# iris-ua/iris_lama

Hardware: AMD Instinct MI355X
Metric: particle-scans/sec (higher is better)
Workload: dtype f64; 1 GPU; PFSlam2D 30 particles, 1080-beam synthetic corridor log (SURVEY.md 8(d)), res 0.05 m, patch 32, l2_max 0.5, GN+Cauchy(0.15), seed 42; particles=30, beams=1080, parallelism=particle-shard x1

## Files before the change

### iris_lama_amd/csrc/lama_dev.h

```cpp
#pragma once
#include <hip/hip_runtime.h>
#include <stdint.h>
#include <cstddef>

#ifdef LAMA_WIDE_DM
#define lama_dev lama_dev_wide
#endif

#include "lama_heap.h"

#ifdef LAMA_WAVE_SIM
#define LAMA_LOCKSTEP() ((void)__ballot(true))
#else
#define LAMA_LOCKSTEP() ((void)0)
#endif

namespace lama_dev {

#ifdef LAMA_WIDE_DM
typedef uint32_t sv_t;
constexpr uint32_t SV_VALID = 0x80000000u;
constexpr uint32_t SV_QUEUED = 0x40000000u;
constexpr uint32_t SV_SQMASK = 0x3FFFFFFFu;
constexpr int SV_VALID_BIT = 31;
constexpr uint32_t MAX_OFFSET_CELLS = 255;
#else
typedef uint16_t sv_t;
constexpr uint16_t SV_VALID = 0x8000;
constexpr uint16_t SV_QUEUED = 0x4000;
constexpr uint16_t SV_SQMASK = 0x3FFF;
constexpr int SV_VALID_BIT = 15;
constexpr uint32_t MAX_OFFSET_CELLS = 127;
#endif
constexpr uint32_t SV_BYTES = (uint32_t)sizeof(sv_t);
constexpr uint32_t SV_PATCH_BYTES = 1024u * SV_BYTES;

// ... 25 lines not shown
    uint32_t qcap;
    const PartRec* part;
    uint32_t max_sqdist;
    uint32_t max_iter;
    double scale, off, resolution, maxdist, meas_sigma;
    double trunc_ray, trunc_range;
    int16_t* dm_dir;
    int16_t* occ_dir;
    int32_t* counts;
    double* poses;
    uint64_t* q_lower;
    uint64_t* q_raise;
    uint32_t* qsizes;
    uint32_t* slow;
    uint32_t* slow_list;
    uint32_t* slow_n;
    uint8_t* heavy;
    const uint32_t* elist;
    const uint32_t* elist_n;
    const uint8_t* early;
    uint32_t lane;
    uint64_t* act;
    uint32_t* act_count;
    uint32_t act_cap;
    uint64_t* stats;
    int32_t* err;
    uint64_t* dbg;
    uint32_t* guard;
    uint32_t guard_r;
    uint32_t occ_policy, ray_rule;
    uint32_t strategy;
    double lo_miss, lo_hit, lo_min, lo_max;
};

struct PV {
    int16_t* dm_dir; int16_t* occ_dir;
    sv_t* dm_sv; uint32_t* dm_obs; uint64_t* dm_mask;
    uint32_t* occ; uint64_t* occ_mask; uint64_t* occ_hit;
    int32_t* counts; int32_t* rev;
    uint32_t dm_cap, occ_cap;
};
#ifdef LAMA_WAVE_SIM
__device__ inline uint32_t part_u32(const uint32_t* q) { return *q; }
__device__ inline uint64_t part_u64(const uint64_t* q) { return *q; }
#else
__device__ inline uint32_t part_u32(const uint32_t* q)
{
    return (uint32_t)__builtin_amdgcn_readfirstlane((int)__hip_atomic_load(q, __ATOMIC_RELAXED, __HIP_MEMORY_SCOPE_AGENT));
}
__device__ inline uint64_t part_u64(const uint64_t* q)
{
    const uint64_t v = __hip_atomic_load(q, __ATOMIC_RELAXED, __HIP_MEMORY_SCOPE_AGENT);
    const uint32_t lo = (uint32_t)__builtin_amdgcn_readfirstlane((int)(uint32_t)v), hi = (uint32_t)__builtin_amdgcn_readfirstlane((int)(uint32_t)(v >> 32));
    return ((uint64_t)hi << 32) | lo;
}
#endif
#if defined(LAMA_KC_PROBE) && !defined(LAMA_WAVE_SIM)
__device__ uint32_t g_kc_n;
__device__ uint64_t g_kc_ev[64][8];
__device__ __noinline__ void kc_probe(const DevParams& prm, int p)
{
    const uint64_t* q = reinterpret_cast<const uint64_t*>(prm.part + p);
#if LAMA_KC_PROBE == 2
    __builtin_amdgcn_s_dcache_inv();
#endif
    const unsigned long long act = __ballot(1);
// ... 423 lines not shown
```

### iris_lama_amd/csrc/lama_hip.hip

```cpp
#include "../../include/lama_hip.h"

#include <hip/hip_runtime.h>

#include <algorithm>
#include <cmath>
#include <cstdio>
#include <cstdlib>
#include <cstring>
#include <map>
#include <memory>
#include <mutex>
#include <string>
#include <vector>

#include "lama_kernels.h"
#include "lama_pgo.h"
#include "lama_pgo_pcg.h"
#include "lama_map_build.h"
#include "lama_match_batch.h"
#include "lama_correlative.h"
#include "../host/pgo_pattern.hpp"

using namespace lama_dev;

// ... 841 lines not shown
    return regrid_window(c, (uint32_t)newW, nox, noy);
}

int32_t start_without_first_scan(lama_hip_ctx* c)
{
    if (c->initialised) return LAMA_HIP_OK;
    for (uint32_t p = 0; p < c->P; ++p) { c->h_poses[4 * p] = 1.0; c->h_poses[4 * p + 1] = 0.0; c->h_poses[4 * p + 2] = 0.0; c->h_poses[4 * p + 3] = 0.0; }
    HIPCHK(c, hipMemcpyAsync(c->d_poses, c->h_poses.data(), sizeof(double) * 4 * c->P, hipMemcpyHostToDevice, c->stream));
    c->initialised = true;
    return LAMA_HIP_OK;
}

int32_t fit_window(lama_hip_ctx* c, const Affine& mtf, uint32_t first, uint32_t count)
{
    double far = c->scan_reach;
    if (c->cfg.ray_rule == 0 && c->cfg.truncated_range > 0.0) far = std::min(far, c->cfg.truncated_range);
    const uint32_t guard_r = ((uint32_t)std::ceil(std::sqrt((double)c->max_sqdist)) + 1u + 31u) / 32u;
    const double reach = far + std::sqrt(mtf.t[0] * mtf.t[0] + mtf.t[1] * mtf.t[1]) + (double)(guard_r + 1u) * 32.0 * c->cfg.resolution;
    double xlo = 1e300, xhi = -1e300, ylo = 1e300, yhi = -1e300;
    for (uint32_t p = first; p < first + count; ++p) {
        const double x = c->h_poses[4 * p + 2], y = c->h_poses[4 * p + 3];
        xlo = std::min(xlo, x - reach); xhi = std::max(xhi, x + reach);
        ylo = std::min(ylo, y - reach); yhi = std::max(yhi, y + reach);
    }
    auto patch = [&](double w) { return (int64_t)std::floor((c->scale * w + c->off) / 32.0); };
    return ensure_window(c, patch(xlo), patch(xhi), patch(ylo), patch(yhi));
}

static unsigned xcd_grid(const lama_hip_ctx* c, uint32_t first, uint32_t count)
{
    return first + count == c->P ? (count + 7u) / 8u * 8u : count;
}

int32_t launch_allocation_phase(lama_hip_ctx* c, const DevParams& prm, uint32_t n, uint32_t first, uint32_t count, int alloc_only, hipStream_t s, const double* d_pts)
{
    const size_t need = (size_t)c->P * n;
    if (need > c->d_rrec.n) {
        c->d_rrec.reset(); c->d_rbbox.reset(); c->d_rchunk.reset();
        hipError_t e = c->d_rrec.alloc(need);
        if (e == hipSuccess) e = c->d_rbbox.alloc(need);
        if (e == hipSuccess) e = c->d_rchunk.alloc((size_t)c->P * ((n + 63) / 64));
        if (e != hipSuccess) { c->d_rrec.reset(); return hip_fail(c, e, "ray buffers"); }
    }
    hipLaunchKernelGGL(k_ray_hits, dim3(xcd_grid(c, first, count), (n + 255) / 256), dim3(256), 0, s, prm, d_pts, (int)n, c->d_tfs, (int)first,
                       c->d_rrec, c->d_rbbox, alloc_only, c->d_rchunk);
    const int rw_seg = count <= 64 ? 4 : 1;
    hipLaunchKernelGGL(k_ray_alloc_walk, dim3(xcd_grid(c, first, count), (n * rw_seg + 255) / 256), dim3(256), 0, s, prm, (const lama_dev::RayRec*)c->d_rrec, (int)n, (int)first, rw_seg);
    double far = c->scan_reach;
    if (c->cfg.truncated_range > 0.0) far = std::min(far, c->cfg.truncated_range);
    const int reach_cells = (int)std::ceil(far * c->scale) + 2;
    hipLaunchKernelGGL(k_occ_reverse_dir, dim3(count), dim3(256), 0, s, prm, (int)first, (const double*)c->d_tfs, reach_cells,
                       c->unguarded_retry ? 1 : 0);
    return LAMA_HIP_OK;
}

static uint32_t route_places(const lama_hip_ctx* c, uint32_t count)
{
    const uint32_t slots = c->num_cus * 12u;
    if (c->route_forced || count >= slots) return c->route_cap;
    return std::min<uint32_t>(c->route_cap, std::max<uint32_t>(8u, (slots - count) / 7u));
}

int32_t run_update_maps(lama_hip_ctx* c, uint32_t n, const Affine& mtf, uint32_t first, uint32_t count, StepGroup* g)
{
    hipStream_t s = g ? g->s : (hipStream_t)c->stream;
    const double* d_pts = g ? (const double*)g->d_pts : (const double*)c->d_pts;
    if (!g) {
        const int32_t rcw = fit_window(c, mtf, first, count);
        if (rcw) return rcw;
        c->last_mtf = mtf; c->last_first = first; c->last_count = count;
        if (c->recover_depth == 0) { c->saved_visit_bound = c->visit_bound; c->saved_ctr = c->ctr; }
    }
    PinVec<double>& tfs = c->h_tfs;
    tfs.resize((size_t)c->P * 12);
    for (uint32_t p = first; p < first + count; ++p) host_scan_tf(&c->h_poses[4 * p], mtf, &tfs[12 * (size_t)p]);
    HIPCHK(c, hipMemcpyAsync(c->d_tfs + 12 * (size_t)first, &tfs[12 * (size_t)first], sizeof(double) * 12 * count, hipMemcpyHostToDevice, s));
    DevParams prm = g ? group_params(c, *g) : make_params(c);
    bool early_lane = false;
    {
        Timer t = g ? Timer(c, g, 1) : Timer(c, &c->ctr.ms_raycast, &c->ctr.launches_raycast);
        if (first == 0 && count == c->P && !g) {
            (void)hipMemsetAsync(c->d_slow_n, 0, 32 + sizeof(uint64_t) * 4 * c->P, c->stream);
        } else {
            (void)hipMemsetAsync(prm.slow_n, 0, 32, s);
            (void)hipMemsetAsync(c->d_stats + 4 * (size_t)first, 0, sizeof(uint64_t) * 4 * count, s);
        }
        bool sequential = c->cfg.sequential_raycast == 1 || c->cfg.occupancy_policy == 1 ||
                          c->cfg.ray_rule == 1;
        if (!sequential && (n > 4096u || (uint64_t)n + 4096u > c->cfg.active_capacity)) sequential = true;
        if (!g && !sequential && (uint64_t)c->visit_bound + n >= 65536u) {
            uint32_t m = 0;
            if (c->initialised) {
                (void)hipMemsetAsync(c->d_scalar, 0, sizeof(uint32_t), c->stream);
                hipLaunchKernelGGL(k_occ_max_visited, dim3(c->P), dim3(256), 0, c->stream, prm, c->d_scalar);
                HIPCHK(c, hipMemcpyAsync(&m, c->d_scalar, sizeof(uint32_t), hipMemcpyDeviceToHost, c->stream));
                HIPCHK(c, hipStreamSynchronize(c->stream));
            }
            c->visit_bound = m;
            if ((uint64_t)m + n >= 65536u) { sequential = true; c->ctr.wrap_guard_scans += 1; }
        }
        if (!g) {
            c->visit_bound = (uint32_t)std::min<uint64_t>((uint64_t)c->visit_bound + n, 65535u);
            if (sequential) c->ctr.sequential_raycast_scans += 1; else c->ctr.parallel_raycast_scans += 1;
        }
        if (!g) c->last_guarded = c->cfg.ray_rule == 0;
        if (!g && !c->last_guarded) {
            const double side = 32.0 * c->cfg.resolution;
            const double rp = c->scan_reach / side + 2.5;
            const uint32_t bound = (uint32_t)std::min(32767.0, std::ceil(3.1416 * rp * rp));
            std::vector<CapRequest> reqs;
            for (uint32_t p = first; p < first + count; ++p) {
                const HostPart& pr = c->h_part[p];
                const uint32_t nd = std::min<uint32_t>(MAX_PATCHES, round_up32((uint32_t)c->h_counts[2 * p] + bound)), no = std::min<uint32_t>(MAX_PATCHES, round_up32((uint32_t)c->h_counts[2 * p + 1] + bound));
                if (nd > pr.dm_cap || no > pr.occ_cap) reqs.push_back(CapRequest{p, std::max(nd, pr.dm_cap), std::max(no, pr.occ_cap)});
            }
            if (!reqs.empty()) {
                const int32_t rg = set_capacities(c, reqs);
                if (rg) return rg;
                prm = make_params(c);
            }
        }
        if (sequential) {
            if (c->last_guarded) { const int32_t ra = launch_allocation_phase(c, prm, n, first, count, 1, c->stream, c->d_pts); if (ra) return ra; }
            hipLaunchKernelGGL(k_raycast, dim3(count), dim3(UM_BLOCK), 0, c->stream, prm, c->d_pts, (int)n, c->d_tfs, (int)first);
        } else {
            const bool two_waves_e = c->cfg.brushfire_waves == 2 || (c->cfg.brushfire_waves == 0 && count <= BF_TW_MAX_PARTICLES);
            early_lane = c->early_on && two_waves_e && c->cfg.brushfire_mode == 0 && first == 0 && count == c->P &&
                         count >= std::max<uint32_t>(c->route_min_count, c->early_min_count) && c->route_cap > 0;
            uint32_t host_n = 0;
            if (early_lane && c->ll_valid) {
                const uint32_t places = route_places(c, count);
                double mean = 0; for (uint32_t p = 0; p < c->P; ++p) mean += c->h_ll[p]; mean /= c->P;
                const double lim = 2.5 * std::min(mean, 0.0) - 5.0;
                std::vector<std::pair<double, uint32_t>> cand;
                for (uint32_t p = 0; p < c->P; ++p) if (c->h_ll[p] < lim) cand.emplace_back(c->h_ll[p], p);
                if (cand.size() > places) { std::partial_sort(cand.begin(), cand.begin() + places, cand.end()); cand.resize(places); }
                c->h_hlist.resize(256);
                for (auto& e : cand) c->h_hlist[host_n++] = e.second;
                if (host_n) HIPCHK(c, hipMemcpyAsync(c->d_hlist, c->h_hlist.data(), sizeof(uint32_t) * host_n, hipMemcpyHostToDevice, c->stream));
            }
            const bool prev_ok = c->early_ok && c->early_candidates > 0;
            early_lane = early_lane && (host_n > 0 || prev_ok);
            if (early_lane)
                hipLaunchKernelGGL(k_early_list, dim3(1), dim3(256), 0, c->stream, prev_ok ? (const uint8_t*)c->d_heavy : (const uint8_t*)nullptr,
                                   (const uint32_t*)c->d_hlist, host_n, c->d_early, c->d_elist, c->d_slow_n + 4, (int)c->P, route_places(c, count));
            { const int32_t ra = launch_allocation_phase(c, prm, n, first, count, 0, s, d_pts); if (ra) return ra; }
#ifdef LAMA_WAVE_SIM
            const unsigned gy = 4u;
#else
            const unsigned gy = count <= 64 ? 128u : (count >= 1024 ? 8u : 32u);
#endif
            if (early_lane) {
                DevParams pe = prm;
                pe.elist = c->d_elist; pe.elist_n = c->d_slow_n + 4; pe.lane = 1;
                const unsigned eg = route_places(c, count);
                hipLaunchKernelGGL(k_ray_patches, dim3(eg, 128u), dim3(256), 0, c->stream, pe, (const lama_dev::RayRec*)c->d_rrec,
                                   (const uint64_t*)c->d_rbbox, (const lama_dev::RayChunk*)c->d_rchunk, (int)n, 0);
                hipLaunchKernelGGL((k_ray_replay<RP_SORT_SMALL, RP_SORT_SMALL, false, RP_BLOCK_LARGE>), dim3(eg), dim3(RP_BLOCK_LARGE), 0, c->stream, pe, 0);
                hipLaunchKernelGGL((k_ray_replay<8192, 8192, true, RP_BLOCK_LARGE>), dim3(eg), dim3(RP_BLOCK_LARGE), 0, c->stream, pe, 0);
                HIPCHK(c, hipEventRecord(c->ev_alloc, c->stream));
                HIPCHK(c, hipStreamWaitEvent(c->stream3, c->ev_alloc, 0));
                hipLaunchKernelGGL(k_mark_early, dim3(1), dim3(64), 0, c->stream3, pe);
                HIPCHK(c, hipEventRecord(c->ev_go, c->stream3));
                hipLaunchKernelGGL((k_brushfire<LQ_BIG, RQ_BIG, true, true>), dim3(eg), dim3(2 * UM_BLOCK), c->big_stage_pad, c->stream3, pe, 0, 2);
                HIPCHK(c, hipEventRecord(c->ev_early, c->stream3));
                HIPCHK(c, hipStreamWaitEvent(c->stream, c->ev_go, 0));
                prm.early = c->d_early;
            }
            hipLaunchKernelGGL(k_ray_patches, dim3(xcd_grid(c, first, count), gy), dim3(256), 0, s, prm, (const lama_dev::RayRec*)c->d_rrec,
                               (const uint64_t*)c->d_rbbox, (const lama_dev::RayChunk*)c->d_rchunk, (int)n, (int)first);
            const unsigned resume_grid = std::min<unsigned>(count, 256u);
            if (count <= 512) {
                hipLaunchKernelGGL((k_ray_replay<RP_SORT_SMALL, RP_SORT_SMALL, false, RP_BLOCK_LARGE>), dim3(count), dim3(RP_BLOCK_LARGE), 0, s, prm, (int)first);
                hipLaunchKernelGGL((k_ray_replay<8192, 8192, true, RP_BLOCK_LARGE>), dim3(resume_grid), dim3(RP_BLOCK_LARGE), 0, s, prm, (int)first);
            } else {
                hipLaunchKernelGGL((k_ray_replay<RP_SORT_SMALL, RP_SORT_SMALL, false, RP_BLOCK_SMALL>), dim3(count), dim3(RP_BLOCK_SMALL), 0, s, prm, (int)first);
                hipLaunchKernelGGL((k_ray_replay<8192, 8192, true, RP_BLOCK_SMALL>), dim3(resume_grid), dim3(RP_BLOCK_SMALL), 0, s, prm, (int)first);
            }
        }
// ... 109 lines not shown
        Timer t(c, &c->ctr.ms_resample, &c->ctr.launches_resample);
        rc = run_jobs(c, true);
        t.stop();
    }
    if (rc) return rc;
    HIPCHK(c, hipMemcpyAsync(c->ms.counts, c->h_counts.data(), sizeof(int32_t) * 2 * P, hipMemcpyHostToDevice, c->stream));
    HIPCHK(c, hipMemcpyAsync(c->d_poses, c->h_poses.data(), sizeof(double) * 4 * P, hipMemcpyHostToDevice, c->stream));
    HIPCHK(c, hipStreamSynchronize(c->stream));
    resolve_timers(c);
    c->ctr.resample_clones += clones.size();
    c->ctr.resample_bytes += c->clone_bytes;
    return LAMA_HIP_OK;
}

int32_t apply_resample(lama_hip_ctx* c, const int32_t* idx)
{
    c->early_ok = false;
    if (c->ll_valid) { std::vector<double> nl(c->P); for (uint32_t i = 0; i < c->P; ++i) nl[i] = c->h_ll[idx[i]]; c->h_ll.swap(nl); }
    return permute_particles(c, idx);
}

bool step_can_group(const lama_hip_ctx* c, uint32_t n)
{
    return c->step_groups > 1 && c->P < c->route_min_count && c->cfg.brushfire_mode == 0 && c->cfg.sequential_raycast != 1 &&
           c->cfg.occupancy_policy != 1 && c->cfg.ray_rule == 0 && n <= 4096u && (uint64_t)n + 4096u <= c->cfg.active_capacity &&
           (uint64_t)c->visit_bound + n < 65536u;
}

int32_t queue_group_match(lama_hip_ctx* c, StepGroup& g, uint32_t n, const Affine& mtf, bool status_only)
{
    const DevParams prm = group_params(c, g);
    hipStream_t s = g.s;
    const double* const d_pts = g.d_pts;
    const uint32_t* const d_words = g.d_words;
    uint8_t* const d_pack = g.d_pack;
    const int first = (int)g.first, count = (int)g.count;
    if (!status_only) {
        HIPCHK(c, hipMemcpyAsync(c->d_poses + 4 * (size_t)g.first, &c->h_poses[4 * (size_t)g.first], sizeof(double) * 4 * g.count, hipMemcpyHostToDevice, s));
        Timer t(c, &g, 0);
        if (c->max_sqdist > (uint32_t)SM_LUT) hipLaunchKernelGGL(k_scan_match<true>, dim3(count), dim3(SM_BLOCK), 0, s, prm, d_pts, (int)n, mtf, c->d_loglik, c->d_iters, first);
        else hipLaunchKernelGGL(k_scan_match<false>, dim3(count), dim3(SM_BLOCK), 0, s, prm, d_pts, (int)n, mtf, c->d_loglik, c->d_iters, first);
        t.stop();
    }
    hipLaunchKernelGGL(k_pack_group, dim3(1), dim3(64), 0, s, prm, (const double*)c->d_loglik, (const int32_t*)c->d_iters, d_words, first, count, d_pack);
    HIPCHK(c, hipGetLastError());
    HIPCHK(c, hipMemcpyAsync(g.h_pack.data(), d_pack, GroupPack(g.count).bytes, hipMemcpyDeviceToHost, g.s));
    HIPCHK(c, hipEventRecord(g.ev_match, g.s));
    return LAMA_HIP_OK;
}

int32_t recover_group(lama_hip_ctx* c, StepGroup& g, int32_t e)
{
    int32_t rc = wait_for_groups(c);
    if (rc) return rc;
    const size_t o = 4 * (size_t)g.first, m = 4 * (size_t)g.count;
    const std::vector<double> now(c->h_poses.data() + o, c->h_poses.data() + o + m);
    std::memcpy(c->h_poses.data() + o, g.upd_poses.data(), sizeof(double) * m);
    const PinVec<double>& scan = g.upd_slot ? c->h_pts2 : c->h_pts;
    HIPCHK(c, c->d_pts.grow((size_t)3 * g.upd_n, (size_t)3 * 2048));
    HIPCHK(c, hipMemcpyAsync(c->d_pts, scan.data(), sizeof(double) * 3 * g.upd_n, hipMemcpyHostToDevice, c->stream));
    const double reach_now = c->scan_reach;
    c->scan_reach = g.upd_reach; c->last_n = g.upd_n;
    c->last_mtf = g.upd_mtf; c->last_first = g.first; c->last_count = g.count; c->last_guarded = true;
    const uint32_t vb = c->visit_bound;
    const lama_hip_counters before = c->ctr;
    c->saved_visit_bound = vb; c->saved_ctr = c->ctr;
    rc = recover_update(c, e);
    c->visit_bound = vb;
    c->ctr.parallel_raycast_scans = before.parallel_raycast_scans; c->ctr.sequential_raycast_scans = before.sequential_raycast_scans;
    c->ctr.ms_raycast = before.ms_raycast; c->ctr.launches_raycast = before.launches_raycast;
    c->ctr.ms_brushfire = before.ms_brushfire; c->ctr.launches_brushfire = before.launches_brushfire;
    c->ctr.bf_longest_chain_sum = before.bf_longest_chain_sum; c->ctr.bf_longest_chain_last = before.bf_longest_chain_last;
    if (rc == LAMA_HIP_OK) { for (uint32_t p = g.first; p < g.first + g.count; ++p) c->h_chain[p] = c->h_stats[4 * (size_t)p + 3]; c->chain_dirty = true; }
    c->scan_reach = reach_now; c->last_n = 0;
    std::memcpy(c->h_poses.data() + o, now.data(), sizeof(double) * m);
    return rc;
}
// ... 301 lines not shown
    c->wx0 = (px - c->W / 2) * 32;
    c->wy0 = (py - c->W / 2) * 32;
    for (uint32_t p = 0; p < c->P; ++p) std::memcpy(&c->h_poses[4 * p], pose0, sizeof(double) * 4);
    HIPCHK(c, hipMemcpyAsync(c->d_poses, c->h_poses.data(), sizeof(double) * 4 * c->P, hipMemcpyHostToDevice, c->stream));
    int32_t rc = upload_scan(c, pts, n);
    if (rc) return rc;
    const Affine mtf = moving_tf(origin3, quat);
    rc = run_update_maps(c, n, mtf, 0, 1);
    if (rc) return rc;
    rc = check_device_errors(c, true, false);
    if (rc) return rc;
    if (c->P > 1) {
        std::vector<int32_t> idx(c->P, 0);
        rc = permute_particles(c, idx.data());
        if (rc) return rc;
    }
    rc = check_device_errors(c, true, false);
    if (rc) return rc;
    c->initialised = true;
    return LAMA_HIP_OK;
}

int32_t lama_hip_pf_scan_match(lama_hip_ctx* c, const double* pts, uint32_t n, const double* origin3, const double* quat,
                               double* poses_out, double* loglik_out, int32_t* iters_out)
{
    if (!c || !pts || n == 0) return LAMA_HIP_E_INVALID;
    ENTER(c);
    if (!c->initialised) return fail(c, LAMA_HIP_E_STATE, "lama_hip_pf_scan_match before lama_hip_pf_init");
    HIPCHK(c, hipSetDevice(c->cfg.device));
    int32_t rc = upload_scan(c, pts, n);
    if (rc) return rc;
    const Affine mtf = moving_tf(origin3, quat);
    DevParams prm = make_params(c);
    {
        Timer t(c, &c->ctr.ms_scan_match, &c->ctr.launches_scan_match);
        if (c->max_sqdist > (uint32_t)SM_LUT) hipLaunchKernelGGL(k_scan_match<true>, dim3(c->P), dim3(SM_BLOCK), 0, c->stream, prm, c->d_pts, (int)n, mtf, c->d_loglik, c->d_iters, 0);
        else hipLaunchKernelGGL(k_scan_match<false>, dim3(c->P), dim3(SM_BLOCK), 0, c->stream, prm, c->d_pts, (int)n, mtf, c->d_loglik, c->d_iters, 0);
        t.stop();
    }
    HIPCHK(c, hipGetLastError());
    c->h_results.resize(c->results_bytes);
    HIPCHK(c, hipMemcpyAsync(c->h_results.data(), c->d_results, c->results_bytes, hipMemcpyDeviceToHost, c->stream));
    rc = check_device_errors(c, false, c->cfg.profile != 0, true);
    if (rc) return rc;
    const uint8_t* r = c->h_results.data();
    std::memcpy(c->h_poses.data(), r, sizeof(double) * 4 * c->P);
    if (poses_out) std::memcpy(poses_out, r, sizeof(double) * 4 * c->P);
    if (loglik_out) std::memcpy(loglik_out, r + sizeof(double) * 4 * c->P, sizeof(double) * c->P);
    if (iters_out) std::memcpy(iters_out, r + sizeof(double) * 5 * c->P, sizeof(int32_t) * c->P);
    c->h_ll.resize(c->P); std::memcpy(c->h_ll.data(), r + sizeof(double) * 4 * c->P, sizeof(double) * c->P); c->ll_valid = true;
    return LAMA_HIP_OK;
}

int32_t lama_hip_pf_resample(lama_hip_ctx* c, const int32_t* sample_idx)
{
    if (!c || !sample_idx) return LAMA_HIP_E_INVALID;
    if (c->poisoned) return fail(c, LAMA_HIP_E_STATE, "the context ran out of device memory in the middle of a resample and cannot continue");
    if (!c->initialised) return fail(c, LAMA_HIP_E_STATE, "lama_hip_pf_resample before lama_hip_pf_init");
    for (uint32_t i = 0; i < c->P; ++i)
        if (sample_idx[i] < 0 || (uint32_t)sample_idx[i] >= c->P) return fail(c, LAMA_HIP_E_INVALID, "sample_idx out of range");
    if (c->groups_busy && !c->resample_deferred) {
        c->deferred_idx.assign(sample_idx, sample_idx + c->P);
        c->resample_deferred = true;
        return LAMA_HIP_OK;
    }
    ENTER(c);
    HIPCHK(c, hipSetDevice(c->cfg.device));
    return apply_resample(c, sample_idx);
}

// ... 1598 lines not shown
```

### iris_lama_amd/csrc/lama_kernels.h

```cpp
#pragma once
#include "lama_dev.h"

namespace lama_dev {

constexpr int SM_BLOCK = 256;
constexpr int UM_BLOCK = 64;
#ifdef LAMA_TEST_SMALL_QUEUES
constexpr int LQ_SMALL = LAMA_TEST_SMALL_QUEUES, RQ_SMALL = LAMA_TEST_SMALL_QUEUES / 4;
#else
constexpr int LQ_SMALL = 1024, RQ_SMALL = 256;
#endif
constexpr int LQ_BIG = 8192, RQ_BIG = 2048;
constexpr uint32_t BF_TW_MAX_PARTICLES = 1u << 30;

template <int CTRL, int ROW_MASK>
__device__ __forceinline__ double dpp_add(double v)
{
    const uint64_t u = (uint64_t)__double_as_longlong(v);
    const uint32_t lo = (uint32_t)__builtin_amdgcn_update_dpp(0, (int)(uint32_t)u, CTRL, ROW_MASK, 0xF, false);
    const uint32_t hi = (uint32_t)__builtin_amdgcn_update_dpp(0, (int)(uint32_t)(u >> 32), CTRL, ROW_MASK, 0xF, false);
    return v + __longlong_as_double((long long)(((uint64_t)hi << 32) | lo));
}

template <int NV>
// ... 279 lines not shown
                } else {
                    sh.mu = sh.mu * sh.v; sh.v = 2 * sh.v;
                    invalid = true;
                }
                sh.reuse = invalid ? 1 : 0;
            }
            if (invalid) {
                stop = lm ? 0 : 1;
                const double mh[3] = {-sh.h[0], -sh.h[1], -sh.h[2]};
                bool ok = true;
                sh.state = se2_exp_mul(mh, sh.state, ok);
                if (!ok) { if (numeric) *numeric = 1; else atomicOr(prm.err, ERR_NUMERIC); }
                sh.tf = scan_tf(sh.state, mtf);
                sh.have_lin = 0;
            } else {
                for (int k = 0; k < NJ; ++k) sh.tot[k] = sh.tot2[k];
                sh.have_lin = 1;
                sh.lin_is_final = 1;
            }
            sh.ctl[1] = stop;
        }
        ++iter;
        __syncthreads();
        SMT(3);
        if (sh.ctl[1]) break;
    }
#ifdef LAMA_PROFILE_SM
    if (threadIdx.x == 0) for (int k = 0; k < 4; ++k) prm.dbg[8 * blockIdx.x + k] = smp[k];
#endif
    return iter;
}
#undef SMT

template <bool BIGSQ>
__global__ __launch_bounds__(SM_BLOCK) __attribute__((amdgpu_num_vgpr(128))) void k_scan_match(DevParams prm, const double* __restrict__ pts, int n, Affine mtf,
                                                          double* __restrict__ loglik_out, int32_t* __restrict__ iters_out, int first_particle)
{
    __shared__ SMShared sh;
    const int p = first_particle + blockIdx.x;
    const PV pv_ = pview_w(prm, p);
    const int16_t* dir = pv_.dm_dir;
    const sv_t* sv = pv_.dm_sv;
    if (threadIdx.x == 0) {
        sh.state = load_pose(prm.poses + 4 * p);
        sh.tf = scan_tf(sh.state, mtf);
        sh.ctl[0] = 0; sh.ctl[1] = 0;
    }
    sm_build_lut(prm, sh.lut);
    __syncthreads();
    uint32_t evals = 0;
    const uint32_t iter = gn_solve<BIGSQ>(prm, dir, sv, pts, n, mtf, sh, evals);
    double loglik;
    if (sh.lin_is_final) {
        loglik = sh.tot[10];
    } else {
        double a2[2];
        {
            const Affine tf = sh.tf;
            eval_beams_res<BIGSQ>(prm, dir, sv, pts, n, tf, a2, sh.lut);
        }
        block_sum<2>(a2, sh.red, sh.tot2);
        loglik = sh.tot2[1];
    }
    ++evals;
    if (threadIdx.x == 0) {
        double* q = prm.poses + 4 * p;
        q[0] = sh.state.c; q[1] = sh.state.s; q[2] = sh.state.tx; q[3] = sh.state.ty;
        loglik_out[p] = loglik;
        iters_out[p] = (int32_t)iter;
        prm.stats[4 * p + 0] = iter;
        prm.stats[4 * p + 1] = evals;
    }
}

__global__ __launch_bounds__(64) void k_pack_group(DevParams prm, const double* __restrict__ loglik, const int32_t* __restrict__ iters,
                                                    const uint32_t* __restrict__ words, int first_particle, int count, uint8_t* __restrict__ out)
{
    double* o_pose = reinterpret_cast<double*>(out);
    double* o_ll = o_pose + 4 * (size_t)count;
    uint64_t* o_st = reinterpret_cast<uint64_t*>(o_ll + count);
    uint32_t* o_guard = reinterpret_cast<uint32_t*>(o_st + 4 * (size_t)count);
    int32_t* o_cnt = reinterpret_cast<int32_t*>(o_guard + count);
    int32_t* o_it = o_cnt + 2 * (size_t)count;
    uint32_t* o_w = reinterpret_cast<uint32_t*>(o_it + count);
    for (int i = threadIdx.x; i < count; i += 64) {
        const int p = first_particle + i;
        for (int k = 0; k < 4; ++k) { o_pose[4 * i + k] = prm.poses[4 * p + k]; o_st[4 * i + k] = prm.stats[4 * p + k]; }
        o_ll[i] = loglik[p];
        o_guard[i] = prm.guard[p];
        o_cnt[2 * i] = prm.counts[2 * p]; o_cnt[2 * i + 1] = prm.counts[2 * p + 1];
        o_it[i] = iters[p];
    }
    if (threadIdx.x < 16) o_w[threadIdx.x] = words[threadIdx.x];
}

__global__ __launch_bounds__(256) void k_match_eval(DevParams prm, int particle, const double* __restrict__ pts, int n, Affine mtf,
                                                     const double* __restrict__ pose, double* __restrict__ r_out, double* __restrict__ j_out,
                                                     int cell_mode )
{
    __shared__ Affine tfs;
    const PV pv_ = pview_w(prm, particle);
    const int16_t* dir = pv_.dm_dir;
    const sv_t* sv = pv_.dm_sv;
    if (threadIdx.x == 0) tfs = load_scan_tf(pose, mtf);
    __syncthreads();
    const Affine tf = tfs;
    const int i = blockIdx.x * 256 + threadIdx.x;
    if (i >= n) return;
    const double px = pts[3 * i], py = pts[3 * i + 1], pz = pts[3 * i + 2];
    double hx, hy;
    hit_xy(tf, px, py, pz, hx, hy);
    if (cell_mode) { r_out[i] = dm_distance_cell(prm, dir, sv, w2m(prm, hx), w2m(prm, hy)); return; }
    double gx, gy;
    r_out[i] = dm_distance(prm, dir, sv, hx, hy, &gx, &gy);
    if (j_out) { j_out[i] = gx; j_out[(size_t)n + i] = gy; j_out[2 * (size_t)n + i] = gy * hx - gx * hy; }
}

__global__ __launch_bounds__(SM_BLOCK) void k_eval_batch(DevParams prm, int particle, const double* __restrict__ pts, int n,
                                                          Affine mtf, const double* __restrict__ poses,
                                                          double* __restrict__ sqnorm_out, double* __restrict__ loglik_out)
{
    __shared__ double red[(SM_BLOCK / 64) * 2];
    __shared__ double tot[2];
    __shared__ Affine tfs;
    const int b = blockIdx.x;
    const PV pv_ = pview_w(prm, particle);
// ... 1932 lines not shown
```

### iris_lama_amd/csrc/lama_raycast_par.h

```cpp
#pragma once
#include "lama_dev.h"

namespace lama_dev {


constexpr int RP_BLOCK_SMALL = 256, RP_BLOCK_LARGE = 1024;
#ifdef LAMA_TEST_SMALL_QUEUES
constexpr int RP_SORT_SMALL = 512;
#else
constexpr int RP_SORT_SMALL = 2048;
#endif

__device__ inline int dir_alloc_one(int16_t* dir, uint32_t pidx, int32_t* count, int cap, int errbit, int32_t* err)
{
    uint32_t* w = reinterpret_cast<uint32_t*>(dir) + (pidx >> 1);
    const int sh = (int)(pidx & 1u) * 16;
    for (uint32_t spins = 0;; ++spins) {
        const uint32_t v = __hip_atomic_load(w, __ATOMIC_RELAXED, __HIP_MEMORY_SCOPE_AGENT);
        const int s = (int)(int16_t)((v >> sh) & 0xFFFFu);
        if (s >= 0) return s;
        if (s == -3) return -1;
        if (spins > (1u << 22)) { atomicOr(err, errbit); return -1; }
        if (s == -1) {
            const uint32_t locked = (v & ~(0xFFFFu << sh)) | (0xFFFEu << sh);
// ... 78 lines not shown
    g.mhx = w2m(prm, hx); g.mhy = w2m(prm, hy);
    g.msx = w2m(prm, sx); g.msy = w2m(prm, sy);
    const uint32_t mhz = w2m(prm, hz), msz = w2m(prm, sz);
    const int64_t d0 = (int64_t)g.mhx - (int64_t)g.msx, d1 = (int64_t)g.mhy - (int64_t)g.msy, d2 = (int64_t)mhz - (int64_t)msz;
    const int64_t a0 = d0 < 0 ? -d0 : d0, a1 = d1 < 0 ? -d1 : d1, a2 = d2 < 0 ? -d2 : d2;
    const int64_t nn = a0 > a1 ? (a0 > a2 ? a0 : a2) : (a1 > a2 ? a1 : a2);
    g.s0 = d0 < 0 ? -1 : 1; g.s1 = d1 < 0 ? -1 : 1;
    g.a0 = (uint32_t)a0; g.a1 = (uint32_t)a1; g.nn = (uint32_t)(nn > 0xFFFFFFFFll ? 0xFFFFFFFFll : nn);
    g.steps = nn > 0 ? (int)g.nn - 1 : 0;
    if (nn >= 8192) g.steps = -1;
    g.magic = (1ull << 42) / (uint64_t)(2 * (nn > 0 && nn < 8192 ? nn : 1)) + 1ull;
    return g;
}

constexpr int ACT_SEQ_BITS = 26, ACT_XY_BITS = 15;
__device__ inline uint64_t act_key(uint32_t rx, uint32_t ry, uint32_t beam, uint32_t t)
{
    return ((uint64_t)((ry << ACT_XY_BITS) | rx) << ACT_SEQ_BITS) | (uint64_t)((beam << 13) | t);
}

__device__ inline void act_append(const DevParams& prm, int p, uint64_t key)
{
    const uint32_t k = atomicAdd(prm.act_count + p, 1u);
    if (k < prm.act_cap) prm.act[(size_t)p * prm.act_cap + k] = key;
    else atomicOr(prm.err, ERR_QUEUE);
}

struct RayRec;
struct RayChunk;
constexpr uint64_t RAY_BBOX_EMPTY = 0x0000FFFF0000FFFFull;
__device__ inline uint64_t ray_hits_record(const DevParams& prm, const BeamGeom& g, int p, int i, int n, RayRec* rec_out, uint64_t* bbox_out);
__device__ inline void ray_chunk_record(const DevParams& prm, const BeamGeom& g, uint64_t bb, int lane, RayChunk* chunks, size_t index);

__global__ __launch_bounds__(256) void k_ray_hits(DevParams prm, const double* __restrict__ pts, int n,
                                                   const double* __restrict__ tfs, int first_particle,
                                                   RayRec* __restrict__ rec_out = nullptr, uint64_t* __restrict__ bbox_out = nullptr, int alloc_only = 0,
                                                   RayChunk* __restrict__ chunk_out = nullptr)
{
    const int p = first_particle + blockIdx.x;
    if (p >= (int)prm.P) return;
    const int i = blockIdx.y * 256 + threadIdx.x;
    const int lane = threadIdx.x & 63;
    const bool live = i < n;
    const int ic = live ? i : n - 1;
    double T[12];
    uload_f64_w<12>(tfs + 12 * (size_t)p, T);
    const BeamGeom g = beam_geometry(prm, T, pts[3 * ic], pts[3 * ic + 1], pts[3 * ic + 2]);
    uint64_t bb = RAY_BBOX_EMPTY;
    if (rec_out && live) bb = ray_hits_record(prm, g, p, i, n, rec_out, bbox_out);
    if (chunk_out && (i & ~63) < n) ray_chunk_record(prm, g, bb, lane, chunk_out, (size_t)p * ((n + 63) / 64) + (i >> 6));
    if (live && g.steps < 0) atomicOr(prm.err, ERR_WINDOW);
    if (!alloc_only) {
        uint32_t st = (live && g.steps > 0) ? (uint32_t)g.steps : 0u;
        for (int off = 32; off > 0; off >>= 1) st += (uint32_t)__shfl_xor((int)st, off, 64);
        if (lane == 0 && st) atomicAdd((unsigned long long*)(prm.stats + 4 * p + 2), (unsigned long long)st);
    }
    bool hit = live && g.steps >= 0 && g.mark_hit;
    const uint32_t rx = g.mhx - prm.wx0, ry = g.mhy - prm.wy0;
    if (hit && (rx >= prm.WC || ry >= prm.WC)) { atomicOr(prm.err, ERR_WINDOW); hit = false; }
    const uint32_t pidx = (ry >> 5) * prm.W + (rx >> 5), ci = (rx & 31u) | ((ry & 31u) << 5);
    int slot = -1;
    const PV pv = pview(prm, p);
    if (hit) slot = dir_get_or_alloc(pv.occ_dir, pidx, prm.counts + 2 * p + 1, (int)pv.occ_cap, ERR_OCC_CAP, prm.err);
    hit = hit && slot >= 0 && !alloc_only;
    if (hit) atomicOr((unsigned long long*)(pv.occ_hit + (size_t)slot * 16 + (ci >> 6)), 1ull << (ci & 63));
    const unsigned long long hm = __ballot(hit);
    if (hm) {
        uint32_t base = 0;
        if (lane == (__ffsll((long long)hm) - 1)) base = atomicAdd(prm.act_count + p, (uint32_t)__popcll(hm));
        base = (uint32_t)__shfl((int)base, __ffsll((long long)hm) - 1, 64);
        if (hit) {
            const uint32_t k = base + (uint32_t)__popcll(hm & ((1ull << lane) - 1ull));
            if (k < prm.act_cap) prm.act[(size_t)p * prm.act_cap + k] = act_key(rx, ry, (uint32_t)i, 0u);
            else atomicOr(prm.err, ERR_QUEUE);
        }
    }
}

template <int RP_BLOCK>
// ... 230 lines not shown
```

### iris_lama_amd/csrc/lama_raycast_patch.h

```cpp
#pragma once
#include "lama_raycast_par.h"

namespace lama_dev {

struct RayRec {
    uint32_t msx, msy;
    uint32_t a01;
    uint32_t nnf;
    uint64_t magic;
};
struct RayChunk {
    int32_t cwx, cwy;
    int32_t ccwx, ccwy;
    uint64_t bbox;
    uint32_t sxy;
    uint32_t cone;
};

__device__ inline RayRec ray_rec(const BeamGeom& g)
{
    RayRec r;
    r.msx = g.msx; r.msy = g.msy;
    r.a01 = (g.a0 & 0xFFFFu) | ((g.a1 & 0xFFFFu) << 16);
    r.nnf = (g.nn & 0xFFFFu) | (g.s0 < 0 ? 1u << 16 : 0u) | (g.s1 < 0 ? 1u << 17 : 0u) | (g.steps > 0 ? 1u << 18 : 0u);
// ... 81 lines not shown
    const int i = g / RW_SEG, seg = g % RW_SEG;
    if (i >= n || p >= (int)prm.P) return;
    const RayRec r = recs[(size_t)p * n + i];
    if (!(r.nnf & (1u << 18))) return;
    const uint32_t steps = (r.nnf & 0xFFFFu) - 1u;
    const uint32_t t0 = 1u + (uint32_t)(((uint64_t)steps * (uint32_t)seg) / RW_SEG), t1 = (uint32_t)(((uint64_t)steps * (uint32_t)(seg + 1)) / RW_SEG);
    const PV pv = pview(prm, p);
    int16_t* occ_dir = pv.occ_dir;
    if (t0 > t1) return;
    const uint32_t a0 = r.a01 & 0xFFFFu, a1 = r.a01 >> 16, nn = r.nnf & 0xFFFFu;
    const uint32_t k0 = (uint32_t)(((uint64_t)(2u * t0 * a0 + nn) * r.magic) >> 42), k1 = (uint32_t)(((uint64_t)(2u * t0 * a1 + nn) * r.magic) >> 42);
    const bool neg0 = (r.nnf >> 16) & 1u, neg1 = (r.nnf >> 17) & 1u;
    const uint32_t bx = r.msx - prm.wx0, by = r.msy - prm.wy0;
    const uint32_t rx = neg0 ? bx - k0 : bx + k0, ry = neg1 ? by - k1 : by + k1;
    uint32_t X = rx >> 5, Y = ry >> 5;
    uint32_t kx = neg0 ? k0 + (rx & 31u) + 1u : k0 + 32u - (rx & 31u), ky = neg1 ? k1 + (ry & 31u) + 1u : k1 + 32u - (ry & 31u);
    auto step_of = [nn](uint32_t k, uint32_t a) { return k > a ? 0xFFFFFFFFu : (2u * nn * k - nn + 2u * a - 1u) / (2u * a); };
    uint32_t tx = step_of(kx, a0), ty = step_of(ky, a1);
    (void)dir_get_or_alloc(occ_dir, Y * prm.W + X, prm.counts + 2 * p + 1, (int)pv.occ_cap, ERR_OCC_CAP, prm.err);
    for (;;) {
        const uint32_t t = tx < ty ? tx : ty;
        if (t > t1) break;
        if (tx == t) { X = neg0 ? X - 1u : X + 1u; kx += 32u; tx = step_of(kx, a0); }
        if (ty == t) { Y = neg1 ? Y - 1u : Y + 1u; ky += 32u; ty = step_of(ky, a1); }
        (void)dir_get_or_alloc(occ_dir, Y * prm.W + X, prm.counts + 2 * p + 1, (int)pv.occ_cap, ERR_OCC_CAP, prm.err);
    }
}

__device__ inline int imin(int a, int b) { return a < b ? a : b; }
__device__ inline int imax(int a, int b) { return a > b ? a : b; }
constexpr int RD_MARK_SIDE = 256;
constexpr int RD_MARK_WORDS = RD_MARK_SIDE * RD_MARK_SIDE / 32;

__global__ __launch_bounds__(256) void k_occ_reverse_dir(DevParams prm, int first_particle,
                                                          const double* __restrict__ tfs , int reach_cells, int guard_off)
{
    __shared__ uint32_t mark[RD_MARK_WORDS];
    __shared__ uint32_t need_s;
    const int p = first_particle + blockIdx.x;
    const uint32_t W = prm.W, WW = W * W;
    const int tid = threadIdx.x, r = (int)prm.guard_r;
    const PV pv = pview_w(prm, p);
    const int16_t* occ_dir = pv.occ_dir;
    const int16_t* dm_dir = pv.dm_dir;
    const int scx = (int)(w2m(prm, uload_f64(tfs + 12 * (size_t)p + 9)) - prm.wx0), scy = (int)(w2m(prm, uload_f64(tfs + 12 * (size_t)p + 10)) - prm.wy0);
    const int bx0 = imax((scx - reach_cells) >> 5, 0), bx1 = imin((scx + reach_cells) >> 5, (int)W - 1);
    const int by0 = imax((scy - reach_cells) >> 5, 0), by1 = imin((scy + reach_cells) >> 5, (int)W - 1);
    const int mx0 = imax(bx0 - r, 0), my0 = imax(by0 - r, 0), mw = imin(bx1 + r, (int)W - 1) - mx0 + 1, mh = imin(by1 + r, (int)W - 1) - my0 + 1;
    const bool bounded = mw > 0 && mh > 0 && mw <= RD_MARK_SIDE && mh <= RD_MARK_SIDE;
    const uint32_t nbits = bounded ? (uint32_t)(mw * mh) : 0u;
    for (uint32_t i = tid; i < (nbits + 31u) / 32u; i += 256u) mark[i] = 0;
    if (tid == 0) need_s = 0;
    __syncthreads();
    for (uint32_t w0 = (uint32_t)tid * 8u; w0 < WW; w0 += 256u * 8u) {
        const uint4 q = *reinterpret_cast<const uint4*>(occ_dir + w0);
        if ((q.x & q.y & q.z & q.w) == 0xFFFFFFFFu) continue;
        const uint32_t ww[4] = {q.x, q.y, q.z, q.w};
        const int wy = (int)(w0 / W), x0 = (int)(w0 % W);
#pragma unroll
        for (int k = 0; k < 8; ++k) {
            const int slot = (int)(int16_t)((ww[k >> 1] >> ((k & 1) * 16)) & 0xFFFFu);
            if (slot < 0) continue;
            pv.rev[slot] = (int32_t)(w0 + (uint32_t)k);
            if (!bounded || x0 + k < bx0 || x0 + k > bx1 || wy < by0 || wy > by1) continue;
            for (int dy = -r; dy <= r; ++dy)
                for (int dx = -r; dx <= r; ++dx) {
                    const int x = x0 + k + dx - mx0, y = wy + dy - my0;
                    if ((uint32_t)x < (uint32_t)mw && (uint32_t)y < (uint32_t)mh) { const uint32_t n = (uint32_t)y * (uint32_t)mw + (uint32_t)x; atomicOr(&mark[n >> 5], 1u << (n & 31u)); }
                }
        }
    }
    __syncthreads();
    uint32_t need = 0;
    for (uint32_t i = tid; i < (nbits + 31u) / 32u; i += 256u) {
        uint32_t m = mark[i];
        while (m) {
            const uint32_t n = i * 32u + (uint32_t)(__ffs((int)m) - 1);
            const uint32_t wx = (uint32_t)mx0 + n % (uint32_t)mw, wy = (uint32_t)my0 + n / (uint32_t)mw;
            if (dm_dir[wy * W + wx] < 0) ++need;
            m &= m - 1u;
        }
    }
    if (need) atomicAdd(&need_s, need);
    __syncthreads();
    const bool tiled = !bounded && mw > 0 && mh > 0;
    if (tiled) {
        for (int ty = my0; ty < my0 + mh; ty += RD_MARK_SIDE)
            for (int tx = mx0; tx < mx0 + mw; tx += RD_MARK_SIDE) {
                const int tw = imin(RD_MARK_SIDE, mx0 + mw - tx), th = imin(RD_MARK_SIDE, my0 + mh - ty);
                const uint32_t tbits = (uint32_t)(tw * th);
                for (uint32_t i = tid; i < (tbits + 31u) / 32u; i += 256u) mark[i] = 0;
                __syncthreads();
                const int ry0 = imax(ty - r, by0), ry1 = imin(ty + th - 1 + r, by1);
                const int rx0 = imax(tx - r, bx0), rx1 = imin(tx + tw - 1 + r, bx1);
                const int nx = rx1 - rx0 + 1, nrow = ry1 - ry0 + 1;
                for (int i = tid; nx > 0 && i < nx * nrow; i += 256) {
                    const int ox = rx0 + i % nx, oy = ry0 + i / nx;
                    if (occ_dir[(uint32_t)oy * W + (uint32_t)ox] < 0) continue;
                    for (int dy = -r; dy <= r; ++dy)
                        for (int dx = -r; dx <= r; ++dx) {
                            const int x = ox + dx - tx, y = oy + dy - ty;
                            if ((uint32_t)x < (uint32_t)tw && (uint32_t)y < (uint32_t)th) { const uint32_t n = (uint32_t)y * (uint32_t)tw + (uint32_t)x; atomicOr(&mark[n >> 5], 1u << (n & 31u)); }
                        }
                }
                __syncthreads();
                uint32_t tneed = 0;
                for (uint32_t i = tid; i < (tbits + 31u) / 32u; i += 256u) {
                    uint32_t m = mark[i];
                    while (m) {
                        const uint32_t n = i * 32u + (uint32_t)(__ffs((int)m) - 1);
                        const uint32_t wx = (uint32_t)tx + n % (uint32_t)tw, wy = (uint32_t)ty + n / (uint32_t)tw;
                        if (dm_dir[wy * W + wx] < 0) ++tneed;
                        m &= m - 1u;
                    }
// ... 207 lines not shown
```

Measured before the change: 17650 particle-scans/s.

## Pass small pose/transform tables as kernel arguments and trim reverse-dir scan

For particle groups of up to 16, poses and scan transforms are now passed by value as kernel arguments instead of going through host-to-device memcpys. Stats and word clearing moves into k_pack_group so grouped steps skip two memsets. k_occ_reverse_dir gains a row range limit taken from the map bounding box, and its need-count loop changes from per-word bit iteration to per-bit striding. Together these aim to cut per-step API calls and DMA latency and to shrink the reverse-directory sweep, at the cost of larger kernel argument blocks and more template instantiations.

```diff
diff --git a/iris_lama_amd/csrc/lama_dev.h b/iris_lama_amd/csrc/lama_dev.h
--- a/iris_lama_amd/csrc/lama_dev.h
+++ b/iris_lama_amd/csrc/lama_dev.h
@@ -2,6 +2,7 @@
 #include <hip/hip_runtime.h>
 #include <stdint.h>
 #include <cstddef>
+#include <type_traits>
 
 #ifdef LAMA_WIDE_DM
 #define lama_dev lama_dev_wide
@@ -93,6 +94,11 @@
     uint32_t strategy;
     double lo_miss, lo_hit, lo_min, lo_max;
 };
+
+constexpr int ARG_BLOCK = 16;
+struct PoseTable { double v[4 * ARG_BLOCK]; };
+struct TfTable { double v[12 * ARG_BLOCK]; };
+struct NoTable {};
 
 struct PV {
     int16_t* dm_dir; int16_t* occ_dir;
diff --git a/iris_lama_amd/csrc/lama_hip.hip b/iris_lama_amd/csrc/lama_hip.hip
--- a/iris_lama_amd/csrc/lama_hip.hip
+++ b/iris_lama_amd/csrc/lama_hip.hip
@@ -897,8 +897,10 @@
     return first + count == c->P ? (count + 7u) / 8u * 8u : count;
 }
 
-int32_t launch_allocation_phase(lama_hip_ctx* c, const DevParams& prm, uint32_t n, uint32_t first, uint32_t count, int alloc_only, hipStream_t s, const double* d_pts)
-{
+int32_t launch_allocation_phase(lama_hip_ctx* c, const DevParams& prm, uint32_t n, uint32_t first, uint32_t count, int alloc_only, hipStream_t s, const double* d_pts,
+                                const lama_dev::TfTable* tab = nullptr)
+{
+    const double* const d_tfs = tab ? nullptr : (const double*)c->d_tfs;
     const size_t need = (size_t)c->P * n;
     if (need > c->d_rrec.n) {
         c->d_rrec.reset(); c->d_rbbox.reset(); c->d_rchunk.reset();
@@ -907,15 +909,26 @@
         if (e == hipSuccess) e = c->d_rchunk.alloc((size_t)c->P * ((n + 63) / 64));
         if (e != hipSuccess) { c->d_rrec.reset(); return hip_fail(c, e, "ray buffers"); }
     }
-    hipLaunchKernelGGL(k_ray_hits, dim3(xcd_grid(c, first, count), (n + 255) / 256), dim3(256), 0, s, prm, d_pts, (int)n, c->d_tfs, (int)first,
-                       c->d_rrec, c->d_rbbox, alloc_only, c->d_rchunk);
+    const dim3 hits_grid(xcd_grid(c, first, count), (n + 255) / 256);
+    if (tab) hipLaunchKernelGGL(k_ray_hits<lama_dev::TfTable>, hits_grid, dim3(256), 0, s, prm, d_pts, (int)n, d_tfs, (int)first,
+                                (lama_dev::RayRec*)c->d_rrec, (uint64_t*)c->d_rbbox, alloc_only, (lama_dev::RayChunk*)c->d_rchunk, *tab);
+    else hipLaunchKernelGGL(k_ray_hits<lama_dev::NoTable>, hits_grid, dim3(256), 0, s, prm, d_pts, (int)n, d_tfs, (int)first,
+                            (lama_dev::RayRec*)c->d_rrec, (uint64_t*)c->d_rbbox, alloc_only, (lama_dev::RayChunk*)c->d_rchunk, lama_dev::NoTable());
     const int rw_seg = count <= 64 ? 4 : 1;
     hipLaunchKernelGGL(k_ray_alloc_walk, dim3(xcd_grid(c, first, count), (n * rw_seg + 255) / 256), dim3(256), 0, s, prm, (const lama_dev::RayRec*)c->d_rrec, (int)n, (int)first, rw_seg);
     double far = c->scan_reach;
     if (c->cfg.truncated_range > 0.0) far = std::min(far, c->cfg.truncated_range);
     const int reach_cells = (int)std::ceil(far * c->scale) + 2;
-    hipLaunchKernelGGL(k_occ_reverse_dir, dim3(count), dim3(256), 0, s, prm, (int)first, (const double*)c->d_tfs, reach_cells,
-                       c->unguarded_retry ? 1 : 0);
+    uint32_t row0 = 0, row1 = c->W - 1;
+    if (c->mb_valid) {
+        const int64_t oy = c->wy0 >> 5, W = c->W;
+        const int64_t lo = std::min(std::max(c->mby0 - oy, (int64_t)0), W - 1), hi = std::min(std::max(c->mby1 - oy, (int64_t)0), W - 1);
+        if (hi >= lo) { row0 = (uint32_t)lo; row1 = (uint32_t)hi; }
+    }
+    if (tab) hipLaunchKernelGGL(k_occ_reverse_dir<lama_dev::TfTable>, dim3(count), dim3(256), 0, s, prm, (int)first, d_tfs, reach_cells,
+                                c->unguarded_retry ? 1 : 0, row0, row1, *tab);
+    else hipLaunchKernelGGL(k_occ_reverse_dir<lama_dev::NoTable>, dim3(count), dim3(256), 0, s, prm, (int)first, d_tfs, reach_cells,
+                            c->unguarded_retry ? 1 : 0, row0, row1, lama_dev::NoTable());
     return LAMA_HIP_OK;
 }
 
@@ -939,14 +952,17 @@
     PinVec<double>& tfs = c->h_tfs;
     tfs.resize((size_t)c->P * 12);
     for (uint32_t p = first; p < first + count; ++p) host_scan_tf(&c->h_poses[4 * p], mtf, &tfs[12 * (size_t)p]);
-    HIPCHK(c, hipMemcpyAsync(c->d_tfs + 12 * (size_t)first, &tfs[12 * (size_t)first], sizeof(double) * 12 * count, hipMemcpyHostToDevice, s));
+    const bool tf_by_value = g && count <= (uint32_t)lama_dev::ARG_BLOCK;
+    lama_dev::TfTable tf_tab = lama_dev::TfTable();
+    if (tf_by_value) std::memcpy(tf_tab.v, &tfs[12 * (size_t)first], sizeof(double) * 12 * count);
+    else HIPCHK(c, hipMemcpyAsync(c->d_tfs + 12 * (size_t)first, &tfs[12 * (size_t)first], sizeof(double) * 12 * count, hipMemcpyHostToDevice, s));
     DevParams prm = g ? group_params(c, *g) : make_params(c);
     bool early_lane = false;
     {
         Timer t = g ? Timer(c, g, 1) : Timer(c, &c->ctr.ms_raycast, &c->ctr.launches_raycast);
         if (first == 0 && count == c->P && !g) {
             (void)hipMemsetAsync(c->d_slow_n, 0, 32 + sizeof(uint64_t) * 4 * c->P, c->stream);
-        } else {
+        } else if (!g) {
             (void)hipMemsetAsync(prm.slow_n, 0, 32, s);
             (void)hipMemsetAsync(c->d_stats + 4 * (size_t)first, 0, sizeof(uint64_t) * 4 * count, s);
         }
@@ -1009,7 +1025,7 @@
             if (early_lane)
                 hipLaunchKernelGGL(k_early_list, dim3(1), dim3(256), 0, c->stream, prev_ok ? (const uint8_t*)c->d_heavy : (const uint8_t*)nullptr,
                                    (const uint32_t*)c->d_hlist, host_n, c->d_early, c->d_elist, c->d_slow_n + 4, (int)c->P, route_places(c, count));
-            { const int32_t ra = launch_allocation_phase(c, prm, n, first, count, 0, s, d_pts); if (ra) return ra; }
+            { const int32_t ra = launch_allocation_phase(c, prm, n, first, count, 0, s, d_pts, tf_by_value ? &tf_tab : nullptr); if (ra) return ra; }
 #ifdef LAMA_WAVE_SIM
             const unsigned gy = 4u;
 #else
@@ -1185,17 +1201,27 @@
     const DevParams prm = group_params(c, g);
     hipStream_t s = g.s;
     const double* const d_pts = g.d_pts;
-    const uint32_t* const d_words = g.d_words;
+    uint32_t* const d_words = g.d_words;
     uint8_t* const d_pack = g.d_pack;
     const int first = (int)g.first, count = (int)g.count;
     if (!status_only) {
-        HIPCHK(c, hipMemcpyAsync(c->d_poses + 4 * (size_t)g.first, &c->h_poses[4 * (size_t)g.first], sizeof(double) * 4 * g.count, hipMemcpyHostToDevice, s));
+        const bool by_value = g.count <= (uint32_t)lama_dev::ARG_BLOCK;
+        lama_dev::PoseTable ptab = lama_dev::PoseTable();
+        if (by_value) std::memcpy(ptab.v, &c->h_poses[4 * (size_t)g.first], sizeof(double) * 4 * g.count);
+        else HIPCHK(c, hipMemcpyAsync(c->d_poses + 4 * (size_t)g.first, &c->h_poses[4 * (size_t)g.first], sizeof(double) * 4 * g.count, hipMemcpyHostToDevice, s));
+        const bool big = c->max_sqdist > (uint32_t)SM_LUT;
+        const lama_dev::NoTable none;
         Timer t(c, &g, 0);
-        if (c->max_sqdist > (uint32_t)SM_LUT) hipLaunchKernelGGL(k_scan_match<true>, dim3(count), dim3(SM_BLOCK), 0, s, prm, d_pts, (int)n, mtf, c->d_loglik, c->d_iters, first);
-        else hipLaunchKernelGGL(k_scan_match<false>, dim3(count), dim3(SM_BLOCK), 0, s, prm, d_pts, (int)n, mtf, c->d_loglik, c->d_iters, first);
+        if (by_value) {
+            if (big) hipLaunchKernelGGL((k_scan_match<true, lama_dev::PoseTable>), dim3(count), dim3(SM_BLOCK), 0, s, prm, d_pts, (int)n, mtf, c->d_loglik, c->d_iters, first, ptab);
+            else hipLaunchKernelGGL((k_scan_match<false, lama_dev::PoseTable>), dim3(count), dim3(SM_BLOCK), 0, s, prm, d_pts, (int)n, mtf, c->d_loglik, c->d_iters, first, ptab);
+        } else {
+            if (big) hipLaunchKernelGGL((k_scan_match<true, lama_dev::NoTable>), dim3(count), dim3(SM_BLOCK), 0, s, prm, d_pts, (int)n, mtf, c->d_loglik, c->d_iters, first, none);
+            else hipLaunchKernelGGL((k_scan_match<false, lama_dev::NoTable>), dim3(count), dim3(SM_BLOCK), 0, s, prm, d_pts, (int)n, mtf, c->d_loglik, c->d_iters, first, none);
+        }
         t.stop();
     }
-    hipLaunchKernelGGL(k_pack_group, dim3(1), dim3(64), 0, s, prm, (const double*)c->d_loglik, (const int32_t*)c->d_iters, d_words, first, count, d_pack);
+    hipLaunchKernelGGL(k_pack_group, dim3(1), dim3(64), 0, s, prm, (const double*)c->d_loglik, (const int32_t*)c->d_iters, d_words, first, count, d_pack, status_only ? 0 : 1);
     HIPCHK(c, hipGetLastError());
     HIPCHK(c, hipMemcpyAsync(g.h_pack.data(), d_pack, GroupPack(g.count).bytes, hipMemcpyDeviceToHost, g.s));
     HIPCHK(c, hipEventRecord(g.ev_match, g.s));
@@ -1563,10 +1589,11 @@
     if (rc) return rc;
     const Affine mtf = moving_tf(origin3, quat);
     DevParams prm = make_params(c);
+    const lama_dev::NoTable none;
     {
         Timer t(c, &c->ctr.ms_scan_match, &c->ctr.launches_scan_match);
-        if (c->max_sqdist > (uint32_t)SM_LUT) hipLaunchKernelGGL(k_scan_match<true>, dim3(c->P), dim3(SM_BLOCK), 0, c->stream, prm, c->d_pts, (int)n, mtf, c->d_loglik, c->d_iters, 0);
-        else hipLaunchKernelGGL(k_scan_match<false>, dim3(c->P), dim3(SM_BLOCK), 0, c->stream, prm, c->d_pts, (int)n, mtf, c->d_loglik, c->d_iters, 0);
+        if (c->max_sqdist > (uint32_t)SM_LUT) hipLaunchKernelGGL((k_scan_match<true, lama_dev::NoTable>), dim3(c->P), dim3(SM_BLOCK), 0, c->stream, prm, c->d_pts, (int)n, mtf, c->d_loglik, c->d_iters, 0, none);
+        else hipLaunchKernelGGL((k_scan_match<false, lama_dev::NoTable>), dim3(c->P), dim3(SM_BLOCK), 0, c->stream, prm, c->d_pts, (int)n, mtf, c->d_loglik, c->d_iters, 0, none);
         t.stop();
     }
     HIPCHK(c, hipGetLastError());
diff --git a/iris_lama_amd/csrc/lama_kernels.h b/iris_lama_amd/csrc/lama_kernels.h
--- a/iris_lama_amd/csrc/lama_kernels.h
+++ b/iris_lama_amd/csrc/lama_kernels.h
@@ -335,9 +335,10 @@
 }
 #undef SMT
 
-template <bool BIGSQ>
+template <bool BIGSQ, class PT>
 __global__ __launch_bounds__(SM_BLOCK) __attribute__((amdgpu_num_vgpr(128))) void k_scan_match(DevParams prm, const double* __restrict__ pts, int n, Affine mtf,
-                                                          double* __restrict__ loglik_out, int32_t* __restrict__ iters_out, int first_particle)
+                                                          double* __restrict__ loglik_out, int32_t* __restrict__ iters_out, int first_particle,
+                                                          PT ptab)
 {
     __shared__ SMShared sh;
     const int p = first_particle + blockIdx.x;
@@ -345,7 +346,10 @@
     const int16_t* dir = pv_.dm_dir;
     const sv_t* sv = pv_.dm_sv;
     if (threadIdx.x == 0) {
-        sh.state = load_pose(prm.poses + 4 * p);
+        if constexpr (std::is_same<PT, PoseTable>::value) {
+            const int b = (int)blockIdx.x & (ARG_BLOCK - 1);
+            sh.state = SE2{ptab.v[4 * b], ptab.v[4 * b + 1], ptab.v[4 * b + 2], ptab.v[4 * b + 3]};
+        } else sh.state = load_pose(prm.poses + 4 * p);
         sh.tf = scan_tf(sh.state, mtf);
         sh.ctl[0] = 0; sh.ctl[1] = 0;
     }
@@ -377,7 +381,7 @@
 }
 
 __global__ __launch_bounds__(64) void k_pack_group(DevParams prm, const double* __restrict__ loglik, const int32_t* __restrict__ iters,
-                                                    const uint32_t* __restrict__ words, int first_particle, int count, uint8_t* __restrict__ out)
+                                                    uint32_t* __restrict__ words, int first_particle, int count, uint8_t* __restrict__ out, int clear)
 {
     double* o_pose = reinterpret_cast<double*>(out);
     double* o_ll = o_pose + 4 * (size_t)count;
@@ -393,8 +397,10 @@
         o_guard[i] = prm.guard[p];
         o_cnt[2 * i] = prm.counts[2 * p]; o_cnt[2 * i + 1] = prm.counts[2 * p + 1];
         o_it[i] = iters[p];
+        if (clear) for (int k = 0; k < 4; ++k) prm.stats[4 * p + k] = 0;
     }
     if (threadIdx.x < 16) o_w[threadIdx.x] = words[threadIdx.x];
+    if (clear && threadIdx.x >= 2 && threadIdx.x < 10) words[threadIdx.x] = 0;
 }
 
 __global__ __launch_bounds__(256) void k_match_eval(DevParams prm, int particle, const double* __restrict__ pts, int n, Affine mtf,
diff --git a/iris_lama_amd/csrc/lama_raycast_par.h b/iris_lama_amd/csrc/lama_raycast_par.h
--- a/iris_lama_amd/csrc/lama_raycast_par.h
+++ b/iris_lama_amd/csrc/lama_raycast_par.h
@@ -134,10 +134,11 @@
 __device__ inline uint64_t ray_hits_record(const DevParams& prm, const BeamGeom& g, int p, int i, int n, RayRec* rec_out, uint64_t* bbox_out);
 __device__ inline void ray_chunk_record(const DevParams& prm, const BeamGeom& g, uint64_t bb, int lane, RayChunk* chunks, size_t index);
 
+template <class TAB>
 __global__ __launch_bounds__(256) void k_ray_hits(DevParams prm, const double* __restrict__ pts, int n,
                                                    const double* __restrict__ tfs, int first_particle,
                                                    RayRec* __restrict__ rec_out = nullptr, uint64_t* __restrict__ bbox_out = nullptr, int alloc_only = 0,
-                                                   RayChunk* __restrict__ chunk_out = nullptr)
+                                                   RayChunk* __restrict__ chunk_out = nullptr, TAB tab = TAB())
 {
     const int p = first_particle + blockIdx.x;
     if (p >= (int)prm.P) return;
@@ -146,7 +147,11 @@
     const bool live = i < n;
     const int ic = live ? i : n - 1;
     double T[12];
-    uload_f64_w<12>(tfs + 12 * (size_t)p, T);
+    if constexpr (std::is_same<TAB, TfTable>::value) {
+        const int b = (int)blockIdx.x & (ARG_BLOCK - 1);
+#pragma unroll
+        for (int k = 0; k < 12; ++k) T[k] = tab.v[12 * b + k];
+    } else uload_f64_w<12>(tfs + 12 * (size_t)p, T);
     const BeamGeom g = beam_geometry(prm, T, pts[3 * ic], pts[3 * ic + 1], pts[3 * ic + 2]);
     uint64_t bb = RAY_BBOX_EMPTY;
     if (rec_out && live) bb = ray_hits_record(prm, g, p, i, n, rec_out, bbox_out);
diff --git a/iris_lama_amd/csrc/lama_raycast_patch.h b/iris_lama_amd/csrc/lama_raycast_patch.h
--- a/iris_lama_amd/csrc/lama_raycast_patch.h
+++ b/iris_lama_amd/csrc/lama_raycast_patch.h
@@ -137,18 +137,23 @@
 constexpr int RD_MARK_SIDE = 256;
 constexpr int RD_MARK_WORDS = RD_MARK_SIDE * RD_MARK_SIDE / 32;
 
+template <class TAB>
 __global__ __launch_bounds__(256) void k_occ_reverse_dir(DevParams prm, int first_particle,
-                                                          const double* __restrict__ tfs , int reach_cells, int guard_off)
+                                                          const double* __restrict__ tfs , int reach_cells, int guard_off,
+                                                          uint32_t row0, uint32_t row1, TAB tab)
 {
     __shared__ uint32_t mark[RD_MARK_WORDS];
     __shared__ uint32_t need_s;
     const int p = first_particle + blockIdx.x;
-    const uint32_t W = prm.W, WW = W * W;
+    const uint32_t W = prm.W;
     const int tid = threadIdx.x, r = (int)prm.guard_r;
     const PV pv = pview_w(prm, p);
     const int16_t* occ_dir = pv.occ_dir;
     const int16_t* dm_dir = pv.dm_dir;
-    const int scx = (int)(w2m(prm, uload_f64(tfs + 12 * (size_t)p + 9)) - prm.wx0), scy = (int)(w2m(prm, uload_f64(tfs + 12 * (size_t)p + 10)) - prm.wy0);
+    double stx, sty;
+    if constexpr (std::is_same<TAB, TfTable>::value) { const int tb = (int)blockIdx.x & (ARG_BLOCK - 1); stx = tab.v[12 * tb + 9]; sty = tab.v[12 * tb + 10]; }
+    else { stx = uload_f64(tfs + 12 * (size_t)p + 9); sty = uload_f64(tfs + 12 * (size_t)p + 10); }
+    const int scx = (int)(w2m(prm, stx) - prm.wx0), scy = (int)(w2m(prm, sty) - prm.wy0);
     const int bx0 = imax((scx - reach_cells) >> 5, 0), bx1 = imin((scx + reach_cells) >> 5, (int)W - 1);
     const int by0 = imax((scy - reach_cells) >> 5, 0), by1 = imin((scy + reach_cells) >> 5, (int)W - 1);
     const int mx0 = imax(bx0 - r, 0), my0 = imax(by0 - r, 0), mw = imin(bx1 + r, (int)W - 1) - mx0 + 1, mh = imin(by1 + r, (int)W - 1) - my0 + 1;
@@ -157,7 +162,8 @@
     for (uint32_t i = tid; i < (nbits + 31u) / 32u; i += 256u) mark[i] = 0;
     if (tid == 0) need_s = 0;
     __syncthreads();
-    for (uint32_t w0 = (uint32_t)tid * 8u; w0 < WW; w0 += 256u * 8u) {
+    const uint32_t w_end = (row1 < W ? row1 + 1u : W) * W;
+    for (uint32_t w0 = row0 * W + (uint32_t)tid * 8u; w0 < w_end; w0 += 256u * 8u) {
         const uint4 q = *reinterpret_cast<const uint4*>(occ_dir + w0);
         if ((q.x & q.y & q.z & q.w) == 0xFFFFFFFFu) continue;
         const uint32_t ww[4] = {q.x, q.y, q.z, q.w};
@@ -177,14 +183,10 @@
     }
     __syncthreads();
     uint32_t need = 0;
-    for (uint32_t i = tid; i < (nbits + 31u) / 32u; i += 256u) {
-        uint32_t m = mark[i];
-        while (m) {
-            const uint32_t n = i * 32u + (uint32_t)(__ffs((int)m) - 1);
-            const uint32_t wx = (uint32_t)mx0 + n % (uint32_t)mw, wy = (uint32_t)my0 + n / (uint32_t)mw;
-            if (dm_dir[wy * W + wx] < 0) ++need;
-            m &= m - 1u;
-        }
+    for (uint32_t n = (uint32_t)tid; n < nbits; n += 256u) {
+        if (!((mark[n >> 5] >> (n & 31u)) & 1u)) continue;
+        const uint32_t wx = (uint32_t)mx0 + n % (uint32_t)mw, wy = (uint32_t)my0 + n / (uint32_t)mw;
+        if (dm_dir[wy * W + wx] < 0) ++need;
     }
     if (need) atomicAdd(&need_s, need);
     __syncthreads();
```

Result: faster. 17830 particle-scans/s (median of 6 runs) (+1.0%).
